# meyer-lab/cmtf-pls

Hardware: AMD Instinct MI355X
Metric: nipals_iters_per_sec (higher is better)
Workload: dtype f32

## Files before the change

### cmtf_pls_amd/_lib.py

```python
from __future__ import annotations

import ctypes
import os
from ctypes import c_char_p, c_double, c_int, c_int64, c_size_t, c_uint64, c_void_p

_HERE = os.path.dirname(os.path.abspath(__file__))
LIB_PATH = os.environ.get("CMTFPLS_LIB") or os.path.join(_HERE, "lib", "libcmtfpls.so")

_P = c_void_p

class XcovBlock(ctypes.Structure):
    _fields_ = [("S", _P), ("S2", _P), ("colcnt", _P), ("n_samples", c_double), ("order", c_int), ("A", c_int), ("B", c_int),
                ("n_squarings", c_int), ("Z", _P), ("wA", _P), ("wB", _P), ("info", _P)]


class KfoldState(ctypes.Structure):
    _fields_ = [("I", c_int), ("A", c_int), ("B", c_int), ("M", c_int), ("K", c_int), ("R", c_int)] + [
        (name, _P) for name in ("fold_of", "S", "mean", "Yk", "Gy", "WA", "WB", "Q", "Wa", "Wb", "T", "Gt", "coef", "Rm", "tm",
                                "Tout", "vec", "n_iter", "status", "part")]


SIGNATURES = {
    "cmtfpls_xcov_iterate_blocks_f64": (c_int, [ctypes.POINTER(XcovBlock), c_int, c_int, _P, _P, _P, _P, _P, c_int, _P, c_size_t, _P]),
    "cmtfpls_abi_version": (c_int, []),
    "cmtfpls_last_error": (c_char_p, []),
    "cmtfpls_clear_error": (c_int, []),
    "cmtfpls_status_to_host": (c_int, [_P, _P, c_size_t, _P, _P]),
    "cmtfpls_colstats_workspace_bytes": (c_size_t, [c_int64, c_int64]),
    "cmtfpls_colstats_f32": (c_int, [_P, c_int64, c_int64, _P, _P, _P, c_size_t, _P]),
    "cmtfpls_colstats_f64": (c_int, [_P, c_int64, c_int64, _P, _P, _P, c_size_t, _P]),
    "cmtfpls_sweep_partials": (c_int, []),
    "cmtfpls_center_f32": (c_int, [_P, c_int64, c_int64, _P, _P, _P, _P]),
    "cmtfpls_center_f64": (c_int, [_P, c_int64, c_int64, _P, _P, _P, _P]),
    "cmtfpls_mode0_contract_workspace_bytes": (c_size_t, [c_int64, c_int64]),
    "cmtfpls_mode0_contract_f32": (c_int, [_P, c_int64, c_int64, _P, _P, c_int, _P, c_size_t, _P]),
    "cmtfpls_mode0_contract_f64": (c_int, [_P, c_int64, c_int64, _P, _P, c_int, _P, c_size_t, _P]),
    "cmtfpls_mode0_contract_yq_f32": (c_int, [_P, c_int64, c_int64, _P, c_int, c_int, _P, _P, c_int, _P, c_size_t, _P]),
    "cmtfpls_mode0_contract_yq_f64": (c_int, [_P, c_int64, c_int64, _P, c_int, c_int, _P, _P, c_int, _P, c_size_t, _P]),
    "cmtfpls_colscale_f64": (c_int, [_P, c_int64, _P, c_double, _P]),
    "cmtfpls_rank1_workspace_bytes": (c_size_t, [c_int, c_int]),
    "cmtfpls_rank1_score_f64": (c_int, [_P, c_int, c_int, _P, _P, _P, c_int, _P, c_int, _P, _P, c_size_t, _P]),
    "cmtfpls_rank1_f64": (c_int, [_P, c_int, c_int, _P, _P, _P, _P, c_int, _P, c_size_t, _P]),
    "cmtfpls_rank1_launches_f64": (c_int, [_P, c_int, c_int, _P, _P, _P, _P, c_int, _P, c_size_t, _P]),
    "cmtfpls_rank1_chain_enable": (None, [c_int]),
    "cmtfpls_rank1_chain_enabled": (c_int, []),
    "cmtfpls_normalize_f64": (c_int, [_P, c_int64, _P, _P]),
    "cmtfpls_rank1_tensor_workspace_bytes": (c_size_t, [_P, c_int]),
    "cmtfpls_rank1_tensor_f64": (c_int, [_P, _P, c_int, c_double, _P, c_int, _P, c_int, _P, c_size_t, _P]),
    "cmtfpls_kron_f64": (c_int, [_P, c_int, _P, c_int, _P, _P]),
    "cmtfpls_xcov_workspace_bytes": (c_size_t, [c_int64, c_int64, c_int]),
    "cmtfpls_xcov_f32": (c_int, [_P, c_int64, c_int64, _P, c_int, c_int, _P, c_int, _P, c_size_t, _P]),
    "cmtfpls_xcov_f64": (c_int, [_P, c_int64, c_int64, _P, c_int, c_int, _P, c_int, _P, c_size_t, _P]),
    "cmtfpls_quadform_f64": (c_int, [_P, c_int, _P, _P, _P, _P]),
    "cmtfpls_xcov_iterate_f64": (c_int, [_P, c_int, c_int, c_int, _P, _P, _P, _P, _P, c_int, _P, _P, _P, c_int, _P, c_size_t, _P, c_size_t, _P]),
    "cmtfpls_s_downdate_f64": (c_int, [_P, c_int, c_int, c_int, _P, _P, _P, _P, _P, _P]),
    "cmtfpls_project_rows_f32": (c_int, [_P, c_int64, c_int, c_int, c_int, _P, _P, _P, _P, c_int, _P]),
    "cmtfpls_project_rows_f64": (c_int, [_P, c_int64, c_int, c_int, c_int, _P, _P, _P, _P, c_int, _P]),
    "cmtfpls_project_rows2_f32": (c_int, [_P, c_int, c_int, _P, _P, _P, _P, c_int, c_int, _P, _P, _P, c_int64, c_int, _P, c_int, _P]),
    "cmtfpls_project_rows2_f64": (c_int, [_P, c_int, c_int, _P, _P, _P, _P, c_int, c_int, _P, _P, _P, c_int64, c_int, _P, c_int, _P]),
    "cmtfpls_project_rows_idx_f32": (c_int, [_P, _P, c_int64, c_int, c_int, c_int, _P, _P, _P, _P, c_int, _P]),
    "cmtfpls_project_rows_idx_f64": (c_int, [_P, _P, c_int64, c_int, c_int, c_int, _P, _P, _P, _P, c_int, _P]),
    "cmtfpls_project_rows2_idx_f32": (c_int, [_P, c_int, c_int, _P, _P, _P, _P, c_int, c_int, _P, _P, _P, _P, c_int64, c_int, _P, c_int, _P]),
    "cmtfpls_project_rows2_idx_f64": (c_int, [_P, c_int, c_int, _P, _P, _P, _P, c_int, c_int, _P, _P, _P, _P, c_int64, c_int, _P, c_int, _P]),
    "cmtfpls_allreduce_sum_f64": (c_int, [_P, _P, c_size_t, _P]),
    "cmtfpls_allreduce_sum_f32": (c_int, [_P, _P, c_size_t, _P]),
    "cmtfpls_axpy_scalar_f64": (c_int, [_P, c_int64, _P, _P, _P]),
    "cmtfpls_xcov_deflate_f32": (c_int, [_P, c_int64, c_int, c_int, _P, c_int, c_int, _P, _P, _P, _P, _P, _P, c_size_t, _P]),
    "cmtfpls_xcov_deflate_f64": (c_int, [_P, c_int64, c_int, c_int, _P, c_int, c_int, _P, _P, _P, _P, _P, _P, c_size_t, _P]),
# ... 120 lines not shown
```

### cmtf_pls_amd/backend.py

```python
from __future__ import annotations

import ctypes
from typing import Optional, Tuple

import torch

from . import _lib

_SUFFIX = {torch.float32: "f32", torch.float64: "f64"}


def _ptr(t: Optional[torch.Tensor]):
    return None if t is None else t.data_ptr()


class HipBackend:
    name = "hip"

    def __init__(self, device: Optional[torch.device] = None):
        self.lib = _lib.load()
        if not torch.cuda.is_available():
            raise _lib.CmtfplsError("cmtf_pls_amd needs a ROCm GPU (torch.cuda.is_available() is False); there is no CPU fallback")
        self.device = torch.device(device) if device is not None else torch.device("cuda", torch.cuda.current_device())
        self.n_partials = int(self.lib.cmtfpls_sweep_partials())
        self._ws = {}
        self._status_slots = {}
        self.rank1_squarings = 30
        self.rank1_chain_side = 256 if self.lib.cmtfpls_rank1_chain_enabled() else 0

    def _stream(self):
        return torch.cuda.current_stream(self.device).cuda_stream

    def _workspace(self, key: str, nbytes: int) -> torch.Tensor:
        buf = self._ws.get(key)
        if buf is None or buf.numel() < nbytes:
            buf = torch.empty(max(int(nbytes), 256), dtype=torch.uint8, device=self.device)
            self._ws[key] = buf
        return buf

    def clear_error(self) -> bool:
        return bool(self.lib.cmtfpls_clear_error())

    def empty(self, *shape, dtype=torch.float64) -> torch.Tensor:
        return torch.empty(*shape, dtype=dtype, device=self.device)

    def zeros(self, *shape, dtype=torch.float64) -> torch.Tensor:
        return torch.zeros(*shape, dtype=dtype, device=self.device)

    def _fn(self, base: str, X: torch.Tensor):
        if X.dtype not in _SUFFIX:
            raise TypeError(f"X must be float32 or float64 on device, got {X.dtype}")
        assert X.is_contiguous() and X.device == self.device
        return getattr(self.lib, f"cmtfpls_{base}_{_SUFFIX[X.dtype]}")

    def _close_partials(self, part: torch.Tensor) -> torch.Tensor:
        out = self.empty(1)
        _lib.check(self.lib.cmtfpls_sum_f64(_ptr(part), part.numel(), _ptr(out), self._stream()), "sum")
        return out

    def ceiling(self, op: str, buf: torch.Tensor, row_bytes: int = 0, blocks: int = 2048,
# ... 31 lines not shown
    def mode0_contract(self, X2: torch.Tensor, u: torch.Tensor, masked: bool, out: Optional[torch.Tensor] = None) -> torch.Tensor:
        I, P = X2.shape
        ws = self._workspace("contract", self.lib.cmtfpls_mode0_contract_workspace_bytes(I, P))
        Z = out if out is not None else self.empty(P)
        _lib.check(self._fn("mode0_contract", X2)(_ptr(X2), I, P, _ptr(u), _ptr(Z), int(masked), _ptr(ws), ws.numel(), self._stream()), "mode0_contract")
        return Z

    def mode0_contract_yq(self, X2: torch.Tensor, Y: torch.Tensor, q: torch.Tensor, masked: bool,
                          out: torch.Tensor) -> Optional[torch.Tensor]:
        I, P = X2.shape
        ws = self._workspace("contract", self.lib.cmtfpls_mode0_contract_workspace_bytes(I, P))
        rc = self._fn("mode0_contract_yq", X2)(_ptr(X2), I, P, _ptr(Y), Y.stride(0), Y.shape[1], _ptr(q), _ptr(out), int(masked),
                                               _ptr(ws), ws.numel(), self._stream())
        if rc == 4:
            return None
        _lib.check(rc, "mode0_contract_yq")
        return out

    def colscale(self, Z: torch.Tensor, colcnt: torch.Tensor, n_samples: float) -> None:
        _lib.check(self.lib.cmtfpls_colscale_f64(_ptr(Z), Z.numel(), _ptr(colcnt), float(n_samples), self._stream()), "colscale")

    def rank1(self, Z: torch.Tensor, A: int, B: int, wA: torch.Tensor, wB: torch.Tensor,
              info: Optional[torch.Tensor] = None, n_squarings: Optional[int] = None, launches: bool = False) -> None:
        ws = self._workspace("rank1", self.lib.cmtfpls_rank1_workspace_bytes(A, B))
        fn = self.lib.cmtfpls_rank1_launches_f64 if launches else self.lib.cmtfpls_rank1_f64
        _lib.check(fn(_ptr(Z), A, B, _ptr(wA), _ptr(wB), None, _ptr(info), int(n_squarings or self.rank1_squarings),
                      _ptr(ws), ws.numel(), self._stream()), "rank1")

    def rank1_chain_gave_up(self) -> None:
        self.lib.cmtfpls_rank1_chain_enable(0)
        self.rank1_chain_side = 0

    def rank1_tensor(self, Z: torch.Tensor, dims, tol: float, factors: torch.Tensor,
                     info: Optional[torch.Tensor] = None, n_squarings: Optional[int] = None) -> None:
        import ctypes
        arr = (ctypes.c_int * len(dims))(*[int(d) for d in dims])
        ws = self._workspace("rank1t", self.lib.cmtfpls_rank1_tensor_workspace_bytes(arr, len(dims)))
        _lib.check(self.lib.cmtfpls_rank1_tensor_f64(_ptr(Z), arr, len(dims), float(tol), _ptr(factors), factors.stride(0), _ptr(info),
                                                     int(n_squarings or self.rank1_squarings), _ptr(ws), ws.numel(), self._stream()),
                   "rank1_tensor")

    def kron(self, a: torch.Tensor, b: torch.Tensor, out: torch.Tensor) -> torch.Tensor:
        _lib.check(self.lib.cmtfpls_kron_f64(_ptr(a), a.numel(), _ptr(b), b.numel(), _ptr(out), self._stream()), "kron")
        return out

    def normalize(self, v: torch.Tensor) -> None:
        _lib.check(self.lib.cmtfpls_normalize_f64(_ptr(v), v.numel(), None, self._stream()), "normalize")

    def xcov(self, X2: torch.Tensor, Y: torch.Tensor, masked: bool, out: Optional[torch.Tensor] = None,
             mixed: bool = False) -> Optional[torch.Tensor]:
        I, P = X2.shape
        M = Y.shape[1]
        ws = self._workspace("contract", self.lib.cmtfpls_xcov_workspace_bytes(I, P, M))
        S = out if out is not None else self.empty(M, P)
        fn = self.lib.cmtfpls_xcov_f32_mixed if (mixed and X2.dtype == torch.float32) else self._fn("xcov", X2)
        _lib.check(fn(_ptr(X2), I, P, _ptr(Y), Y.stride(0), M, _ptr(S), int(masked), _ptr(ws), ws.numel(), self._stream()), "xcov")
        return S

    def xcov_deflate(self, X2: torch.Tensor, A: int, B: int, Y: torch.Tensor, t: torch.Tensor, wA: torch.Tensor, wB: torch.Tensor,
                     out: torch.Tensor) -> Optional[torch.Tensor]:
        I, P = X2.shape
        M = Y.shape[1]
        if M > 64 or P % 4 != 0 or P != A * B:
            return None
        ws = self._workspace("contract", self.lib.cmtfpls_xcov_ssq_workspace_bytes(I, P, M))
        ssq = self.empty(1)
        rc = self._fn("xcov_deflate", X2)(_ptr(X2), I, A, B, _ptr(Y), Y.stride(0), M, _ptr(t), _ptr(wA), _ptr(wB), _ptr(out), _ptr(ssq),
                                          _ptr(ws), ws.numel(), self._stream())
        if rc == 4:
            return None
        _lib.check(rc, "xcov_deflate")
        return ssq

    def rank1_score(self, Z: torch.Tensor, A: int, B: int, wA: torch.Tensor, wB: torch.Tensor, S: torch.Tensor, tq: torch.Tensor,
                    info: Optional[torch.Tensor] = None, n_squarings: Optional[int] = None) -> torch.Tensor:
        M = S.shape[0]
        assert S.is_contiguous() and S.shape[1] == A * B and tq.numel() >= M
        ws = self._workspace("rank1", self.lib.cmtfpls_rank1_workspace_bytes(A, B))
        _lib.check(self.lib.cmtfpls_rank1_score_f64(_ptr(Z), A, B, _ptr(wA), _ptr(wB), _ptr(info),
                                                    int(n_squarings if n_squarings is not None else self.rank1_squarings),
                                                    _ptr(S), M, _ptr(tq), _ptr(ws), ws.numel(), self._stream()), "rank1_score")
        return tq

    def xcov_ssq(self, X2: torch.Tensor, Y: torch.Tensor, mean: torch.Tensor, out: torch.Tensor):
        I, P = X2.shape
        M = Y.shape[1]
        ws = self._workspace("contract", self.lib.cmtfpls_xcov_ssq_workspace_bytes(I, P, M))
        ssq = self.empty(1)
        assert mean.is_contiguous() and mean.numel() == P and mean.dtype == torch.float64
        _lib.check(self._fn("xcov_ssq", X2)(_ptr(X2), I, P, _ptr(Y), Y.stride(0), M, _ptr(out), _ptr(mean), _ptr(ssq), _ptr(ws), ws.numel(),
                                            self._stream()), "xcov_ssq")
        return out, ssq

    def xcov_stats(self, X2: torch.Tensor, Y: torch.Tensor, out: torch.Tensor):
        I, P = X2.shape
        M = Y.shape[1]
        if M > 64 or not X2.is_contiguous():
            return None
        ws = self._workspace("contract", self.lib.cmtfpls_xcov_stats_workspace_bytes(I, P, M))
        stats = self.empty(2 * P)
        rc = self._fn("xcov_stats", X2)(_ptr(X2), I, P, _ptr(Y), Y.stride(0), M, _ptr(out), _ptr(stats), _ptr(ws), ws.numel(), self._stream())
# ... 2 lines not shown
        _lib.check(rc, "xcov_stats")
        return out, stats

    def status_snapshot(self, status: torch.Tensor, slot: int, slots: Optional[dict] = None):
        slots = self._status_slots if slots is None else slots
        ent = slots.get((slot, status.numel()))
        if ent is None:
            host, ev = torch.empty(status.numel(), dtype=torch.float64, pin_memory=True), torch.cuda.Event()
            ev.record(torch.cuda.current_stream(self.device))
            ent = slots[(slot, status.numel())] = (host, ev, host.numpy(), host.data_ptr(), ev.cuda_event, status.numel() * 8)
        rc = self.lib.cmtfpls_status_to_host(status.data_ptr(), ent[3], ent[5], ent[4], self._stream())
        if rc:
            _lib.check(rc, "status_to_host")
        return ent

    def status_wait(self, token) -> "np.ndarray":
        token[1].synchronize()
        return token[2]

    def xcov_iterate_plan(self, S: torch.Tensor, A: int, B: int, q_cur: torch.Tensor, Z: torch.Tensor, wA: torch.Tensor,
                          wB: torch.Tensor, status: torch.Tensor, q_new: torch.Tensor, G: torch.Tensor):
        M, P = S.shape
        wc = self._workspace("contract", self.lib.cmtfpls_mode0_contract_workspace_bytes(M, P))
        wr = self._workspace("rank1", self.lib.cmtfpls_rank1_workspace_bytes(A, B))
        keep = (S, q_cur, Z, wA, wB, status, q_new, G, wc, wr)
        fn = self.lib.cmtfpls_xcov_iterate_f64
        head = (_ptr(S), M, A, B, _ptr(q_cur), _ptr(Z), _ptr(wA), _ptr(wB), status[1:3].data_ptr())
        tail = (_ptr(wc), wc.numel(), _ptr(wr), wr.numel())
        qn, Gp, du2 = _ptr(q_new), _ptr(G), status[0:1].data_ptr()
        stream = self._stream

        def enqueue(n_squarings: int, first: bool, _keep=keep) -> None:
            rc = fn(*head, n_squarings, qn, Gp, du2, 1 if first else 0, *tail, stream())
            if rc:
                _lib.check(rc, "xcov_iterate")
        return enqueue

    def xcov_iterate(self, S: torch.Tensor, A: int, B: int, q_cur: torch.Tensor, Z: torch.Tensor, wA: torch.Tensor,
                     wB: torch.Tensor, info: torch.Tensor, n_squarings: int, q_new: torch.Tensor, G: torch.Tensor,
                     du2: torch.Tensor, first: bool) -> None:
        M, P = S.shape
        wc = self._workspace("contract", self.lib.cmtfpls_mode0_contract_workspace_bytes(M, P))
        wr = self._workspace("rank1", self.lib.cmtfpls_rank1_workspace_bytes(A, B))
        _lib.check(self.lib.cmtfpls_xcov_iterate_f64(_ptr(S), M, A, B, _ptr(q_cur), _ptr(Z), _ptr(wA), _ptr(wB), _ptr(info),
                                                     int(n_squarings), _ptr(q_new), _ptr(G), _ptr(du2), int(first),
                                                     _ptr(wc), wc.numel(), _ptr(wr), wr.numel(), self._stream()), "xcov_iterate")

    def xcov_blocks_plan(self, blocks, M: int, q_cur: torch.Tensor, tq: torch.Tensor, q_new: torch.Tensor, G: torch.Tensor,
                         status: torch.Tensor):
        nb = len(blocks)
        if M > 64 or any(b["order"] not in (2, 3) for b in blocks) or tq.numel() != nb * M or not tq.is_contiguous():
            return None
        arr = (_lib.XcovBlock * nb)()
        need = 256
        for i, b in enumerate(blocks):
            for name in ("S", "S2", "colcnt", "Z", "wA", "wB"):
                t = b.get(name)
                assert t is None or (t.is_contiguous() and t.dtype == torch.float64 and t.device == self.device), name
                setattr(arr[i], name, _ptr(t))
            arr[i].n_samples, arr[i].order, arr[i].A, arr[i].B = float(b["n_samples"]), int(b["order"]), int(b["A"]), int(b["B"])
            arr[i].info = status[1 + 2 * i: 3 + 2 * i].data_ptr()
            if b["order"] == 3:
                need = max(need, self.lib.cmtfpls_rank1_workspace_bytes(b["A"], b["B"]))
        wr = self._workspace("rank1", need)
        keep = (blocks, q_cur, tq, q_new, G, status, wr, arr)
        fn, stream = self.lib.cmtfpls_xcov_iterate_blocks_f64, self._stream
# ... 519 lines not shown
```

### cmtf_pls_amd/csrc/rank1.hip

```cpp
#include "common.hpp"
#include <atomic>

namespace cmtfpls {

constexpr int kTile = 16;
constexpr int kMaxTiles = 256;
constexpr int kMaxSteps = 48;

struct Rank1Ctl {
  int done;
  int final_buf;
  int steps_used;
  int last_step;
  double pad[6];
};
__host__ __device__ __forceinline__ size_t rank1_ctl_bytes(int nt) {
  return sizeof(Rank1Ctl) + ((size_t)(kMaxSteps + 2) * nt + 2 * (size_t)nt * nt) * sizeof(double);
}
__device__ __forceinline__ double* ctl_trace(Rank1Ctl* c, int nt, int step) { return reinterpret_cast<double*>(c + 1) + (size_t)step * nt; }
__device__ __forceinline__ double* ctl_fro(Rank1Ctl* c, int nt, int which) {
  return reinterpret_cast<double*>(c + 1) + (size_t)(kMaxSteps + 2) * nt + (size_t)which * nt * nt;
}

__device__ __forceinline__ double pow2_scale_from_trace(const double* parts, int nt, double* tr_out) {
  double tr = 0.0;
  for (int i = 0; i < nt; ++i) tr += parts[i];
  *tr_out = tr;
  if (!(tr > 0.0) || !isfinite(tr)) return 1.0;
  int e;
  frexp(tr, &e);
  return ldexp(1.0, -e);
}

typedef double d4r_t __attribute__((ext_vector_type(4)));

__global__ __launch_bounds__(kTile* kTile) void syrk_step_kernel(const double* __restrict__ M, int n, int k, int ld,
                                                                double* __restrict__ C, Rank1Ctl* __restrict__ ctl,
// ... 112 lines not shown
      double t = 0.0;
      for (int l = 0; l < kTile; ++l) t += diag[l];
      ctl_trace(ctl, nt, step)[blockIdx.x] = t;
    }
  }
}

constexpr unsigned long long kChainEmpty = ~0ull;
constexpr int kChainMaxSteps = 31;
constexpr int kChainSpin = 1 << 15;

__device__ __forceinline__ double chain_ld(const double* p) {
  return __longlong_as_double((long long)__hip_atomic_load(reinterpret_cast<const unsigned long long*>(p), __ATOMIC_RELAXED, __HIP_MEMORY_SCOPE_AGENT));
}
__device__ __forceinline__ void chain_st(double* p, double v) {
  unsigned long long b = (unsigned long long)__double_as_longlong(v);
  if (b == kChainEmpty) b = 0x7FF8000000000000ull;
  __hip_atomic_store(reinterpret_cast<unsigned long long*>(p), b, __ATOMIC_RELAXED, __HIP_MEMORY_SCOPE_AGENT);
}
__device__ __forceinline__ bool chain_empty(double v) { return (unsigned long long)__double_as_longlong(v) == kChainEmpty; }

__global__ __launch_bounds__(256) void chain_preset_kernel(unsigned long long* __restrict__ p, int64_t n) {
  for (int64_t i = (int64_t)blockIdx.x * 256 + threadIdx.x; i < n; i += (int64_t)gridDim.x * 256) p[i] = kChainEmpty;
}

#ifdef CMTFPLS_CHAIN_PROFILE
__device__ unsigned long long g_chain_prof[1024];
#define CHAIN_STAMP(slot) do { if (first_wg && tid == 0 && step < 32) g_chain_prof[step * 8 + (slot)] = __builtin_amdgcn_s_memrealtime(); } while (0)
#define CHAIN_COUNT(slot, v) do { if (first_wg && tid == 0 && step < 32) g_chain_prof[step * 8 + (slot)] = (unsigned long long)(v); } while (0)
#else
#define CHAIN_STAMP(slot) do { } while (0)
#define CHAIN_COUNT(slot, v) do { } while (0)
#endif

__global__ __launch_bounds__(kTile* kTile) void syrk_chain_kernel(const double* __restrict__ M0, int n, int k0,
                                                                 double* gbufs, double* trs, double* fros, double* gave_up,
                                                                 Rank1Ctl* __restrict__ ctl, int n_squarings) {
  constexpr int KC = 128, KW = 8, LDP = KC + 2;
  __shared__ __attribute__((aligned(16))) double pan[2][kTile][LDP];
  __shared__ double red[2][4][kTile * kTile];
  __shared__ double diag[2][kTile];
  __shared__ double fsum[2][4];
  __shared__ double cfro[2][4];
  __shared__ double ctr[2][kTile];
  __shared__ int cdead[2];
  const int tx = threadIdx.x, ty = threadIdx.y, tid = ty * kTile + tx;
// ... 142 lines not shown
    __syncthreads();
    if (tid == 0) {
      chain_st(fros + (int64_t)step * nt2 + blockIdx.y * nt + blockIdx.x, ((fsum[par][0] + fsum[par][1]) + fsum[par][2]) + fsum[par][3]);
      if (blockIdx.x == blockIdx.y) {
        double t = 0.0;
        for (int l = 0; l < kTile; ++l) t += diag[par][l];
        chain_st(trs + (int64_t)step * nt + blockIdx.x, t);
      }
    }
    CHAIN_STAMP(6);
  }
}

__global__ __launch_bounds__(256) void transpose_kernel(const double* __restrict__ Z, int A, int B, double* __restrict__ Zt) {
  const int64_t idx = (int64_t)blockIdx.x * 256 + threadIdx.x;
  if (idx >= (int64_t)A * B) return;
  const int b = (int)(idx / A), a = (int)(idx % A);
  Zt[idx] = Z[(int64_t)a * B + b];
}

__global__ __launch_bounds__(256) void rank1_seed_xy_kernel(const double* __restrict__ M, int n, int k,
                                                           const double* __restrict__ gbase, int64_t gstride,
                                                           const double* __restrict__ G0,
                                                           const Rank1Ctl* __restrict__ ctl, int last_buf, int ny_blocks,
                                                           double* __restrict__ y, double* __restrict__ x) {
  extern __shared__ double seed[];
  __shared__ double red[16];
  __shared__ double rsum[8][33];
  __shared__ double bestv[4];
  __shared__ int besti[4];
  const int fb = (ctl->final_buf >= 0) ? ctl->final_buf : last_buf;
  const double* G = gbase + (int64_t)fb * gstride;
  double bv = -1.0;
  int bi = 0;
  for (int i = threadIdx.x; i < n; i += 256) {
    const double d = G[(int64_t)i * n + i];
    if (d > bv) { bv = d; bi = i; }
  }
#pragma unroll
  for (int m = 32; m > 0; m >>= 1) {
    const double ov = __shfl_xor(bv, m, 64);
    const int oi = __shfl_xor(bi, m, 64);
    if (ov > bv || (ov == bv && oi < bi)) { bv = ov; bi = oi; }
  }
  if ((threadIdx.x & 63) == 0) { bestv[threadIdx.x >> 6] = bv; besti[threadIdx.x >> 6] = bi; }
  __syncthreads();
  bv = bestv[0];
  bi = besti[0];
  for (int w = 1; w < 4; ++w)
    if (bestv[w] > bv || (bestv[w] == bv && besti[w] < bi)) { bv = bestv[w]; bi = besti[w]; }
  double ss = 0.0;
  for (int i = threadIdx.x; i < n; i += 256) {
    const double g = G[(int64_t)bi * n + i];
    seed[i] = g;
    ss = fma(g, g, ss);
// ... 9 lines not shown
      for (int i = lane; i < n; i += 64) s = fma(G0[(int64_t)j * n + i], seed[i], s);
      s = wave_sum(s);
      if (lane == 0) x[j] = s;
    }
    return;
  }
  const int cx = threadIdx.x & 31, ry = threadIdx.x >> 5;
  const int c = blockIdx.x * 32 + cx;
  double s = 0.0;
  if (c < k)
    for (int j = ry; j < n; j += 8) s = fma(M[(int64_t)j * k + c], seed[j], s);
  rsum[ry][cx] = s;
  __syncthreads();
  if (ry == 0 && c < k) {
    double tot = 0.0;
#pragma unroll
    for (int g = 0; g < 8; ++g) tot += rsum[g][cx];
    y[c] = tot;
  }
}

__device__ __forceinline__ void rank1_write_info(double* __restrict__ info, const Rank1Ctl* __restrict__ ctl, const double* gave) {
  if (!info) return;
  if (gave && !chain_empty(chain_ld(gave))) { info[0] = 0.0; info[1] = -1.0; return; }
  info[0] = (ctl->done || ctl->last_step >= 0) ? 1.0 : 0.0;
  info[1] = (double)ctl->steps_used;
}

__device__ __forceinline__ void rank1_final_body(const double* x, const double* y,
                                                 int n, int k, int x_is_A, const Rank1Ctl* __restrict__ ctl,
                                                 double* __restrict__ wA, double* __restrict__ wB,
                                                 double* __restrict__ sigma, double* __restrict__ info, const double* gave) {
  __shared__ double red[2][16];
  __shared__ double bestv[16];
  __shared__ int besti[16];
  double sx = 0.0, sy = 0.0;
  for (int i = threadIdx.x; i < n; i += 1024) sx = fma(x[i], x[i], sx);
  for (int i = threadIdx.x; i < k; i += 1024) sy = fma(y[i], y[i], sy);
  const double nx = sqrt(block_sum(sx, red[0]));
  const double ny = sqrt(block_sum(sy, red[1]));
  const double* vb = x_is_A ? y : x;
  const int nb = x_is_A ? k : n;
  double bv = -1.0;
  int bi = 0;
  for (int i = threadIdx.x; i < nb; i += 1024) {
    const double d = fabs(vb[i]);
    if (d > bv) { bv = d; bi = i; }
  }
#pragma unroll
  for (int m = 32; m > 0; m >>= 1) {
    const double ov = __shfl_xor(bv, m, 64);
    const int oi = __shfl_xor(bi, m, 64);
    if (ov > bv || (ov == bv && oi < bi)) { bv = ov; bi = oi; }
  }
  if ((threadIdx.x & 63) == 0) { bestv[threadIdx.x >> 6] = bv; besti[threadIdx.x >> 6] = bi; }
  __syncthreads();
  bv = bestv[0];
  bi = besti[0];
  for (int w = 1; w < 16; ++w)
    if (bestv[w] > bv || (bestv[w] == bv && besti[w] < bi)) { bv = bestv[w]; bi = besti[w]; }
  const bool gv = gave && !chain_empty(chain_ld(gave));
  const double sgn = gv ? __longlong_as_double(0x7FF8000000000000ll) : ((vb[bi] < 0.0) ? -1.0 : 1.0);
  double* ox = x_is_A ? wA : wB;
  double* oy = x_is_A ? wB : wA;
  for (int i = threadIdx.x; i < n; i += 1024) ox[i] = sgn * (x[i] / nx);
  for (int i = threadIdx.x; i < k; i += 1024) oy[i] = sgn * (y[i] / ny);
  if (threadIdx.x == 0) {
    if (sigma) sigma[0] = nx / ny;
    rank1_write_info(info, ctl, gave);
  }
}

__global__ __launch_bounds__(1024) void rank1_final_kernel(const double* __restrict__ x, const double* __restrict__ y,
                                                          int n, int k, int x_is_A, const Rank1Ctl* __restrict__ ctl,
                                                          double* __restrict__ wA, double* __restrict__ wB,
                                                          double* __restrict__ sigma, double* __restrict__ info, const double* gave) {
  rank1_final_body(x, y, n, k, x_is_A, ctl, wA, wB, sigma, info, gave);
}

__global__ __launch_bounds__(1024) void rank1_final_score_kernel(const double* __restrict__ x, const double* __restrict__ y,
                                                                int n, int k, int x_is_A, const Rank1Ctl* __restrict__ ctl,
                                                                double* __restrict__ wA, double* __restrict__ wB,
                                                                double* __restrict__ info, const double* __restrict__ S, int A, int B,
                                                                double* __restrict__ t, const double* gave) {
  extern __shared__ double lds[];
  __shared__ double red[2][16];
  __shared__ double bestv[16];
  __shared__ int besti[16];
  double* sA = lds;
  double* sB = lds + ((A + 1) & ~1);
  double sx = 0.0, sy = 0.0;
  for (int i = threadIdx.x; i < n; i += 1024) sx = fma(x[i], x[i], sx);
  for (int i = threadIdx.x; i < k; i += 1024) sy = fma(y[i], y[i], sy);
  const double nx = sqrt(block_sum(sx, red[0]));
  const double ny = sqrt(block_sum(sy, red[1]));
  const double* vb = x_is_A ? y : x;
  const int nb = x_is_A ? k : n;
  double bv = -1.0;
  int bi = 0;
  for (int i = threadIdx.x; i < nb; i += 1024) {
    const double d = fabs(vb[i]);
    if (d > bv) { bv = d; bi = i; }
  }
#pragma unroll
  for (int m = 32; m > 0; m >>= 1) {
    const double ov = __shfl_xor(bv, m, 64);
    const int oi = __shfl_xor(bi, m, 64);
    if (ov > bv || (ov == bv && oi < bi)) { bv = ov; bi = oi; }
  }
  if ((threadIdx.x & 63) == 0) { bestv[threadIdx.x >> 6] = bv; besti[threadIdx.x >> 6] = bi; }
  __syncthreads();
  bv = bestv[0];
  bi = besti[0];
  for (int w = 1; w < 16; ++w)
    if (bestv[w] > bv || (bestv[w] == bv && besti[w] < bi)) { bv = bestv[w]; bi = besti[w]; }
  const bool gv = gave && !chain_empty(chain_ld(gave));
  const double sgn = gv ? __longlong_as_double(0x7FF8000000000000ll) : ((vb[bi] < 0.0) ? -1.0 : 1.0);
  double* lx = x_is_A ? sA : sB;
  double* ly = x_is_A ? sB : sA;
  double* ox = x_is_A ? wA : wB;
  double* oy = x_is_A ? wB : wA;
  const bool store = blockIdx.x == 0;
  for (int i = threadIdx.x; i < n; i += 1024) {
    const double v = sgn * (x[i] / nx);
    lx[i] = v;
    if (store) ox[i] = v;
  }
  for (int i = threadIdx.x; i < k; i += 1024) {
    const double v = sgn * (y[i] / ny);
    ly[i] = v;
    if (store) oy[i] = v;
  }
  if (store && threadIdx.x == 0) rank1_write_info(info, ctl, gave);
  __syncthreads();
  using VT = Pack<double, 2>;
  const int64_t P = (int64_t)A * B;
  const int64_t step = (int64_t)1024 * 2;
  const double* __restrict__ xr = S + (int64_t)blockIdx.x * P;
  KronWalk w((int64_t)threadIdx.x * 2, step, B);
// ... 9 lines not shown
      double d = 0.0;
      d = fma(xs[u].e[0], sB[w.k], d);
      d = fma(xs[u].e[1], sB[w.k + 1], d);
      acc = fma(sA[w.j], d, acc);
      w.next();
    }
  }
  for (; c < P; c += step) {
    const VT xv = ld_stream(reinterpret_cast<const VT*>(xr + c));
    double d = 0.0;
    d = fma(xv.e[0], sB[w.k], d);
    d = fma(xv.e[1], sB[w.k + 1], d);
    acc = fma(sA[w.j], d, acc);
    w.next();
  }
  acc = block_sum(acc, red[0]);
  if (threadIdx.x == 0) t[blockIdx.x] = acc;
}

static inline size_t align_up(size_t x, size_t a) { return (x + a - 1) / a * a; }

static std::atomic<int> g_chain_on{1};

static int chain_slots() {
  static int slots = 0;
  if (slots == 0) {
    int dev = 0, cus = 0;
    if (hipGetDevice(&dev) != hipSuccess || hipDeviceGetAttribute(&cus, hipDeviceAttributeMultiprocessorCount, dev) != hipSuccess || cus <= 0) cus = 256;
    slots = 2 * cus;
  }
  return slots;
}

}

using namespace cmtfpls;

extern "C" {

size_t cmtfpls_rank1_workspace_bytes(int A, int B) {
  if (A <= 0 || B <= 0) return 0;
  const size_t n = (size_t)(A < B ? A : B), k = (size_t)(A < B ? B : A);
  const size_t nt = (n + kTile - 1) / kTile;
  const size_t chain = nt * nt <= 256 ? align_up(((size_t)(kChainMaxSteps + 1) * (n * n + nt + nt * nt) + 1) * sizeof(double), 256) : 0;
  return align_up(rank1_ctl_bytes((int)nt), 256) + 3 * align_up(n * n * sizeof(double), 256) +
         align_up((size_t)A * B * sizeof(double), 256) + align_up(n * sizeof(double), 256) + align_up(k * sizeof(double), 256) + chain;
}

static int rank1_run(const double* Z, int A, int B, double* wA, double* wB, double* sigma, double* info,
                     int n_squarings, void* ws, size_t ws_bytes, void* stream, const double* S, int M, double* tq, bool allow_chain = true);

int cmtfpls_rank1_f64(const double* Z, int A, int B, double* wA, double* wB, double* sigma, double* info,
                      int n_squarings, void* ws, size_t ws_bytes, void* stream) {
  return rank1_run(Z, A, B, wA, wB, sigma, info, n_squarings, ws, ws_bytes, stream, nullptr, 0, nullptr);
}

#ifdef CMTFPLS_CHAIN_PROFILE
int cmtfpls_debug_chain_prof(unsigned long long* out) { return (int)hipMemcpyFromSymbol(out, HIP_SYMBOL(g_chain_prof), sizeof(unsigned long long) * 1024); }
#endif
void cmtfpls_rank1_chain_enable(int on) { g_chain_on.store((on == 1 || on == 2) ? on : 0, std::memory_order_relaxed); }
int cmtfpls_rank1_chain_enabled(void) { return g_chain_on.load(std::memory_order_relaxed); }

int cmtfpls_rank1_launches_f64(const double* Z, int A, int B, double* wA, double* wB, double* sigma, double* info,
                               int n_squarings, void* ws, size_t ws_bytes, void* stream) {
  return rank1_run(Z, A, B, wA, wB, sigma, info, n_squarings, ws, ws_bytes, stream, nullptr, 0, nullptr, false);
}

int cmtfpls_rank1_score_f64(const double* Z, int A, int B, double* wA, double* wB, double* info, int n_squarings,
                            const double* S, int M, double* tq, void* ws, size_t ws_bytes, void* stream) {
  if (!S || !tq || M <= 0) { set_error("rank1_score: bad argument"); return CMTFPLS_EINVAL; }
  const int64_t P = (int64_t)A * B;
  if (M > 64 || P < 8192 || (B % 2) != 0 || ((size_t)(((A + 1) & ~1) + B) * sizeof(double)) > 60 * 1024 ||
      (reinterpret_cast<uintptr_t>(S) & 15) != 0) {
    int rc = cmtfpls_rank1_f64(Z, A, B, wA, wB, nullptr, info, n_squarings, ws, ws_bytes, stream);
    if (rc == CMTFPLS_OK) rc = cmtfpls_score_s_f64(S, M, A, B, wA, wB, tq, stream);
    return rc;
  }
  return rank1_run(Z, A, B, wA, wB, nullptr, info, n_squarings, ws, ws_bytes, stream, S, M, tq);
}

static int rank1_run(const double* Z, int A, int B, double* wA, double* wB, double* sigma, double* info,
                     int n_squarings, void* ws, size_t ws_bytes, void* stream, const double* S, int M, double* tq, bool allow_chain) {
  if (!Z || !wA || !wB || A <= 0 || B <= 0) { set_error("rank1: bad argument"); return CMTFPLS_EINVAL; }
  const int n = A < B ? A : B, k = A < B ? B : A;
  if (n > kTile * kMaxTiles) { set_error("rank1: min(A, B) > 4096 unsupported"); return CMTFPLS_EUNSUPPORTED; }
  if ((size_t)n * sizeof(double) > 64 * 1024) { set_error("rank1: seed exceeds the LDS"); return CMTFPLS_EUNSUPPORTED; }
  if (n_squarings < 1) n_squarings = 1;
  if (n_squarings > kMaxSteps) n_squarings = kMaxSteps;
  if (!ws || ws_bytes < cmtfpls_rank1_workspace_bytes(A, B)) { set_error("rank1: workspace too small"); return CMTFPLS_EWORKSPACE; }
  hipStream_t st = (hipStream_t)stream;
  char* p = static_cast<char*>(ws);
  Rank1Ctl* ctl = reinterpret_cast<Rank1Ctl*>(p);
  p += align_up(rank1_ctl_bytes((n + kTile - 1) / kTile), 256);
  double* buf0 = reinterpret_cast<double*>(p);
  p += align_up((size_t)n * n * sizeof(double), 256);
  double* buf1 = reinterpret_cast<double*>(p);
  p += align_up((size_t)n * n * sizeof(double), 256);
  double* g0keep = reinterpret_cast<double*>(p);
  p += align_up((size_t)n * n * sizeof(double), 256);
  double* Zt = reinterpret_cast<double*>(p);
  p += align_up((size_t)A * B * sizeof(double), 256);
  double* xv = reinterpret_cast<double*>(p);
  p += align_up((size_t)n * sizeof(double), 256);
  double* yv = reinterpret_cast<double*>(p);
  p += align_up((size_t)k * sizeof(double), 256);
  double* chain_region = reinterpret_cast<double*>(p);

  const double* M0 = Z;
  if (A > B) {
    const int64_t tot = (int64_t)A * B;
    hipLaunchKernelGGL(transpose_kernel, dim3((unsigned)((tot + 255) / 256)), dim3(256), 0, st, Z, A, B, Zt);
    M0 = Zt;
  }
  const int nt = (n + kTile - 1) / kTile;
  const dim3 grid(nt, nt), block(kTile, kTile);
  const int ny_blocks = (k + 31) / 32;
  const double* gave = nullptr;
  if (allow_chain && g_chain_on.load(std::memory_order_relaxed) && nt * nt <= 256 && nt * nt <= chain_slots() && n_squarings <= kChainMaxSteps) {
    const size_t nn = (size_t)n * n, steps = (size_t)n_squarings + 1;
    double* gbufs = chain_region;
    double* trs = gbufs + steps * nn;
    double* fros = trs + steps * nt;
    double* gave_up = fros + steps * (size_t)nt * nt;
    gave = gave_up;
    const int64_t words = (int64_t)(steps * (nn + nt + (size_t)nt * nt) + 1);
    hipLaunchKernelGGL(chain_preset_kernel, dim3((unsigned)((words + 2047) / 2048)), dim3(256), 0, st, reinterpret_cast<unsigned long long*>(chain_region), words);
    const dim3 cgrid(nt, (g_chain_on.load(std::memory_order_relaxed) == 2 && nt > 1) ? nt - 1 : nt);
    hipLaunchKernelGGL(syrk_chain_kernel, cgrid, block, 0, st, M0, n, k, gbufs, trs, fros, gave_up, ctl, n_squarings);
    hipLaunchKernelGGL(rank1_seed_xy_kernel, dim3(ny_blocks + (n + 3) / 4), dim3(256), (size_t)n * sizeof(double), st,
                       M0, n, k, gbufs, (int64_t)nn, gbufs, ctl, n_squarings, ny_blocks, yv, xv);
  } else {
    hipLaunchKernelGGL(syrk_step_kernel, grid, block, 0, st, M0, n, k, k, buf0, ctl, 0, 0, g0keep);
    for (int s = 1; s <= n_squarings; ++s) {
      const double* in = (s & 1) ? buf0 : buf1;
      double* out = (s & 1) ? buf1 : buf0;
      hipLaunchKernelGGL(syrk_step_kernel, grid, block, 0, st, in, n, n, n, out, ctl, s, s & 1, (double*)nullptr);
    }
    hipLaunchKernelGGL(rank1_seed_xy_kernel, dim3(ny_blocks + (n + 3) / 4), dim3(256), (size_t)n * sizeof(double), st,
                       M0, n, k, buf0, (int64_t)(buf1 - buf0), g0keep, ctl, n_squarings & 1, ny_blocks, yv, xv);
  }
  if (S) {
    const size_t lds = (size_t)(((A + 1) & ~1) + B) * sizeof(double);
    hipLaunchKernelGGL(rank1_final_score_kernel, dim3((unsigned)M), dim3(1024), lds, st, xv, yv, n, k, (A <= B) ? 1 : 0, ctl, wA, wB, info,
                       S, A, B, tq, gave);
    return check_launch("rank1_score");
  }
  hipLaunchKernelGGL(rank1_final_kernel, dim3(1), dim3(1024), 0, st, xv, yv, n, k, (A <= B) ? 1 : 0, ctl, wA, wB, sigma, info, gave);
  return check_launch("rank1");
}

}
```

### include/cmtfpls.h

```cpp
#ifndef CMTFPLS_H
#define CMTFPLS_H

#include <stddef.h>
#include <stdint.h>

#ifdef __cplusplus
extern "C" {
#endif

#define CMTFPLS_OK 0
#define CMTFPLS_EINVAL 1
#define CMTFPLS_EWORKSPACE 2
#define CMTFPLS_EHIP 3
#define CMTFPLS_EUNSUPPORTED 4

int cmtfpls_abi_version(void);
const char* cmtfpls_last_error(void);
int cmtfpls_clear_error(void);
int cmtfpls_status_to_host(const void* src, void* dst_host, size_t bytes, void* event, void* stream);

size_t cmtfpls_colstats_workspace_bytes(int64_t I, int64_t P);
int cmtfpls_colstats_f32(const float* X, int64_t I, int64_t P, double* colsum, double* colcnt,
                         void* ws, size_t ws_bytes, void* stream);
int cmtfpls_colstats_f64(const double* X, int64_t I, int64_t P, double* colsum, double* colcnt,
// ... 2 lines not shown
int cmtfpls_center_f32(float* X, int64_t I, int64_t P, const double* mean, double* rowcnt,
                       double* ssq_part, void* stream);
int cmtfpls_center_f64(double* X, int64_t I, int64_t P, const double* mean, double* rowcnt,
                       double* ssq_part, void* stream);

size_t cmtfpls_mode0_contract_workspace_bytes(int64_t I, int64_t P);
int cmtfpls_mode0_contract_f32(const float* X, int64_t I, int64_t P, const double* u, double* Z,
                               int masked, void* ws, size_t ws_bytes, void* stream);
int cmtfpls_mode0_contract_f64(const double* X, int64_t I, int64_t P, const double* u, double* Z,
                               int masked, void* ws, size_t ws_bytes, void* stream);
int cmtfpls_mode0_contract_yq_f32(const float* X, int64_t I, int64_t P, const double* Y, int ldy, int M,
                                  const double* q, double* Z, int masked, void* ws, size_t ws_bytes, void* stream);
int cmtfpls_mode0_contract_yq_f64(const double* X, int64_t I, int64_t P, const double* Y, int ldy, int M,
                                  const double* q, double* Z, int masked, void* ws, size_t ws_bytes, void* stream);
int cmtfpls_colscale_f64(double* Z, int64_t P, const double* colcnt, double n_samples, void* stream);

size_t cmtfpls_rank1_workspace_bytes(int A, int B);
int cmtfpls_rank1_f64(const double* Z, int A, int B, double* wA, double* wB, double* sigma, double* info,
                      int n_squarings, void* ws, size_t ws_bytes, void* stream);
int cmtfpls_rank1_launches_f64(const double* Z, int A, int B, double* wA, double* wB, double* sigma, double* info,
                               int n_squarings, void* ws, size_t ws_bytes, void* stream);
void cmtfpls_rank1_chain_enable(int on);
int cmtfpls_rank1_chain_enabled(void);
int cmtfpls_rank1_score_f64(const double* Z, int A, int B, double* wA, double* wB, double* info, int n_squarings,
                            const double* S, int M, double* tq, void* ws, size_t ws_bytes, void* stream);
int cmtfpls_normalize_f64(double* v, int64_t n, double* nrm, void* stream);
size_t cmtfpls_rank1_tensor_workspace_bytes(const int* dims, int n);
int cmtfpls_rank1_tensor_f64(const double* Z, const int* dims, int n, double tol, double* factors, int ld,
                             double* info, int n_squarings, void* ws, size_t ws_bytes, void* stream);
int cmtfpls_kron_f64(const double* a, int na, const double* b, int nb, double* out, void* stream);

size_t cmtfpls_xcov_workspace_bytes(int64_t I, int64_t P, int M);
int cmtfpls_xcov_f32(const float* X, int64_t I, int64_t P, const double* Y, int ldy, int M, double* S,
                     int masked, void* ws, size_t ws_bytes, void* stream);
int cmtfpls_xcov_f64(const double* X, int64_t I, int64_t P, const double* Y, int ldy, int M, double* S,
                     int masked, void* ws, size_t ws_bytes, void* stream);
int cmtfpls_quadform_f64(const double* G, int M, const double* q, const double* q_old, double* out, void* stream);
int cmtfpls_xcov_deflate_f32(float* X, int64_t I, int A, int B, const double* Y, int ldy, int M, const double* t, const double* wA,
                             const double* wB, double* S, double* ssq, void* ws, size_t ws_bytes, void* stream);
int cmtfpls_xcov_deflate_f64(double* X, int64_t I, int A, int B, const double* Y, int ldy, int M, const double* t, const double* wA,
                             const double* wB, double* S, double* ssq, void* ws, size_t ws_bytes, void* stream);
size_t cmtfpls_xcov_ssq_workspace_bytes(int64_t I, int64_t P, int M);
size_t cmtfpls_xcov_stats_workspace_bytes(int64_t I, int64_t P, int M);
int cmtfpls_xcov_stats_f32(const float* X, int64_t I, int64_t P, const double* Y, int ldy, int M, double* S, double* stats,
                           void* ws, size_t ws_bytes, void* stream);
int cmtfpls_xcov_stats_f64(const double* X, int64_t I, int64_t P, const double* Y, int ldy, int M, double* S, double* stats,
// ... 233 lines not shown
```

Measured before the change: 765.6.

## Carry chain-region reset into rank1 final kernel to skip preset launch

Rank1 workspaces are now registered per shape, and the chain-region reset (writing the empty sentinel) is done by extra blocks appended to the final/score kernel. The next call on the same workspace can then skip the separate chain_preset_kernel launch. The gave-up flag is latched into the control block by the seed kernel, because the final kernel now overwrites the region that flag lives in. This removes one kernel launch per rank1 call on the hot NIPALS path, at the cost of host-side mutex/map bookkeeping, special handling under graph capture, and a one-shape-per-workspace restriction.

```diff
diff --git a/cmtf_pls_amd/_lib.py b/cmtf_pls_amd/_lib.py
--- a/cmtf_pls_amd/_lib.py
+++ b/cmtf_pls_amd/_lib.py
@@ -44,6 +44,10 @@
     "cmtfpls_rank1_launches_f64": (c_int, [_P, c_int, c_int, _P, _P, _P, _P, c_int, _P, c_size_t, _P]),
     "cmtfpls_rank1_chain_enable": (None, [c_int]),
     "cmtfpls_rank1_chain_enabled": (c_int, []),
+    "cmtfpls_rank1_workspace_register": (c_int, [_P]),
+    "cmtfpls_rank1_workspace_release": (c_int, [_P]),
+    "cmtfpls_rank1_preset_carry_enable": (None, [c_int]),
+    "cmtfpls_rank1_preset_carry_enabled": (c_int, []),
     "cmtfpls_normalize_f64": (c_int, [_P, c_int64, _P, _P]),
     "cmtfpls_rank1_tensor_workspace_bytes": (c_size_t, [_P, c_int]),
     "cmtfpls_rank1_tensor_f64": (c_int, [_P, _P, c_int, c_double, _P, c_int, _P, c_int, _P, c_size_t, _P]),
diff --git a/cmtf_pls_amd/backend.py b/cmtf_pls_amd/backend.py
--- a/cmtf_pls_amd/backend.py
+++ b/cmtf_pls_amd/backend.py
@@ -1,6 +1,7 @@
 from __future__ import annotations
 
 import ctypes
+import weakref
 from typing import Optional, Tuple
 
 import torch
@@ -12,6 +13,11 @@
 
 def _ptr(t: Optional[torch.Tensor]):
     return None if t is None else t.data_ptr()
+
+
+def _release_rank1_workspaces(lib, ptrs) -> None:
+    for ptr in ptrs:
+        lib.cmtfpls_rank1_workspace_release(ptr)
 
 
 class HipBackend:
@@ -27,6 +33,8 @@
         self._status_slots = {}
         self.rank1_squarings = 30
         self.rank1_chain_side = 256 if self.lib.cmtfpls_rank1_chain_enabled() else 0
+        self._rank1_registered = []
+        weakref.finalize(self, _release_rank1_workspaces, self.lib, self._rank1_registered)
 
     def _stream(self):
         return torch.cuda.current_stream(self.device).cuda_stream
@@ -36,6 +44,15 @@
         if buf is None or buf.numel() < nbytes:
             buf = torch.empty(max(int(nbytes), 256), dtype=torch.uint8, device=self.device)
             self._ws[key] = buf
+        return buf
+
+    def _rank1_workspace(self, A: int, B: int) -> torch.Tensor:
+        key = ("rank1", int(A), int(B))
+        buf = self._ws.get(key)
+        if buf is None:
+            buf = self._ws[key] = torch.empty(max(int(self.lib.cmtfpls_rank1_workspace_bytes(A, B)), 256), dtype=torch.uint8, device=self.device)
+            _lib.check(self.lib.cmtfpls_rank1_workspace_register(buf.data_ptr()), "rank1_workspace_register")
+            self._rank1_registered.append(buf.data_ptr())
         return buf
 
     def clear_error(self) -> bool:
@@ -113,7 +130,7 @@
 
     def rank1(self, Z: torch.Tensor, A: int, B: int, wA: torch.Tensor, wB: torch.Tensor,
               info: Optional[torch.Tensor] = None, n_squarings: Optional[int] = None, launches: bool = False) -> None:
-        ws = self._workspace("rank1", self.lib.cmtfpls_rank1_workspace_bytes(A, B))
+        ws = self._rank1_workspace(A, B)
         fn = self.lib.cmtfpls_rank1_launches_f64 if launches else self.lib.cmtfpls_rank1_f64
         _lib.check(fn(_ptr(Z), A, B, _ptr(wA), _ptr(wB), None, _ptr(info), int(n_squarings or self.rank1_squarings),
                       _ptr(ws), ws.numel(), self._stream()), "rank1")
@@ -121,6 +138,8 @@
     def rank1_chain_gave_up(self) -> None:
         self.lib.cmtfpls_rank1_chain_enable(0)
         self.rank1_chain_side = 0
+        for ptr in self._rank1_registered:
+            self.lib.cmtfpls_rank1_workspace_register(ptr)
 
     def rank1_tensor(self, Z: torch.Tensor, dims, tol: float, factors: torch.Tensor,
                      info: Optional[torch.Tensor] = None, n_squarings: Optional[int] = None) -> None:
@@ -167,7 +186,7 @@
                     info: Optional[torch.Tensor] = None, n_squarings: Optional[int] = None) -> torch.Tensor:
         M = S.shape[0]
         assert S.is_contiguous() and S.shape[1] == A * B and tq.numel() >= M
-        ws = self._workspace("rank1", self.lib.cmtfpls_rank1_workspace_bytes(A, B))
+        ws = self._rank1_workspace(A, B)
         _lib.check(self.lib.cmtfpls_rank1_score_f64(_ptr(Z), A, B, _ptr(wA), _ptr(wB), _ptr(info),
                                                     int(n_squarings if n_squarings is not None else self.rank1_squarings),
                                                     _ptr(S), M, _ptr(tq), _ptr(ws), ws.numel(), self._stream()), "rank1_score")
@@ -216,7 +235,7 @@
                           wB: torch.Tensor, status: torch.Tensor, q_new: torch.Tensor, G: torch.Tensor):
         M, P = S.shape
         wc = self._workspace("contract", self.lib.cmtfpls_mode0_contract_workspace_bytes(M, P))
-        wr = self._workspace("rank1", self.lib.cmtfpls_rank1_workspace_bytes(A, B))
+        wr = self._rank1_workspace(A, B)
         keep = (S, q_cur, Z, wA, wB, status, q_new, G, wc, wr)
         fn = self.lib.cmtfpls_xcov_iterate_f64
         head = (_ptr(S), M, A, B, _ptr(q_cur), _ptr(Z), _ptr(wA), _ptr(wB), status[1:3].data_ptr())
@@ -235,7 +254,7 @@
                      du2: torch.Tensor, first: bool) -> None:
         M, P = S.shape
         wc = self._workspace("contract", self.lib.cmtfpls_mode0_contract_workspace_bytes(M, P))
-        wr = self._workspace("rank1", self.lib.cmtfpls_rank1_workspace_bytes(A, B))
+        wr = self._rank1_workspace(A, B)
         _lib.check(self.lib.cmtfpls_xcov_iterate_f64(_ptr(S), M, A, B, _ptr(q_cur), _ptr(Z), _ptr(wA), _ptr(wB), _ptr(info),
                                                      int(n_squarings), _ptr(q_new), _ptr(G), _ptr(du2), int(first),
                                                      _ptr(wc), wc.numel(), _ptr(wr), wr.numel(), self._stream()), "xcov_iterate")
diff --git a/cmtf_pls_amd/csrc/rank1.hip b/cmtf_pls_amd/csrc/rank1.hip
--- a/cmtf_pls_amd/csrc/rank1.hip
+++ b/cmtf_pls_amd/csrc/rank1.hip
@@ -1,5 +1,7 @@
 #include "common.hpp"
 #include <atomic>
+#include <mutex>
+#include <unordered_map>
 
 namespace cmtfpls {
 
@@ -12,7 +14,9 @@
   int final_buf;
   int steps_used;
   int last_step;
-  double pad[6];
+  int gave_seen;
+  int pad_i;
+  double pad[5];
 };
 __host__ __device__ __forceinline__ size_t rank1_ctl_bytes(int nt) {
   return sizeof(Rank1Ctl) + ((size_t)(kMaxSteps + 2) * nt + 2 * (size_t)nt * nt) * sizeof(double);
@@ -171,6 +175,15 @@
 
 __global__ __launch_bounds__(256) void chain_preset_kernel(unsigned long long* __restrict__ p, int64_t n) {
   for (int64_t i = (int64_t)blockIdx.x * 256 + threadIdx.x; i < n; i += (int64_t)gridDim.x * 256) p[i] = kChainEmpty;
+}
+
+__device__ __forceinline__ void chain_represet(unsigned long long* __restrict__ p, int64_t n, int first) {
+  const int64_t stride = (int64_t)(gridDim.x - first) * blockDim.x;
+  for (int64_t i = (int64_t)((int)blockIdx.x - first) * blockDim.x + threadIdx.x; i < n; i += stride) p[i] = kChainEmpty;
+}
+__host__ __device__ __forceinline__ int chain_represet_blocks(int64_t words) {
+  const int64_t b = (words + 4095) / 4096;
+  return (int)(b < 1 ? 1 : (b > 128 ? 128 : b));
 }
 
 #ifdef CMTFPLS_CHAIN_PROFILE
@@ -359,8 +372,8 @@
 __global__ __launch_bounds__(256) void rank1_seed_xy_kernel(const double* __restrict__ M, int n, int k,
                                                            const double* __restrict__ gbase, int64_t gstride,
                                                            const double* __restrict__ G0,
-                                                           const Rank1Ctl* __restrict__ ctl, int last_buf, int ny_blocks,
-                                                           double* __restrict__ y, double* __restrict__ x) {
+                                                           Rank1Ctl* __restrict__ ctl, int last_buf, int ny_blocks,
+                                                           double* __restrict__ y, double* __restrict__ x, const double* gave) {
   extern __shared__ double seed[];
   __shared__ double red[16];
   __shared__ double rsum[8][33];
@@ -368,6 +381,7 @@
   __shared__ int besti[4];
   const int fb = (ctl->final_buf >= 0) ? ctl->final_buf : last_buf;
   const double* G = gbase + (int64_t)fb * gstride;
+  if (blockIdx.x == 0 && threadIdx.x == 0) ctl->gave_seen = (gave && !chain_empty(chain_ld(gave))) ? 1 : 0;
   double bv = -1.0;
   int bi = 0;
   for (int i = threadIdx.x; i < n; i += 256) {
@@ -423,7 +437,7 @@
 
 __device__ __forceinline__ void rank1_write_info(double* __restrict__ info, const Rank1Ctl* __restrict__ ctl, const double* gave) {
   if (!info) return;
-  if (gave && !chain_empty(chain_ld(gave))) { info[0] = 0.0; info[1] = -1.0; return; }
+  if (gave && ctl->gave_seen) { info[0] = 0.0; info[1] = -1.0; return; }
   info[0] = (ctl->done || ctl->last_step >= 0) ? 1.0 : 0.0;
   info[1] = (double)ctl->steps_used;
 }
@@ -460,7 +474,7 @@
   bi = besti[0];
   for (int w = 1; w < 16; ++w)
     if (bestv[w] > bv || (bestv[w] == bv && besti[w] < bi)) { bv = bestv[w]; bi = besti[w]; }
-  const bool gv = gave && !chain_empty(chain_ld(gave));
+  const bool gv = gave && ctl->gave_seen;
   const double sgn = gv ? __longlong_as_double(0x7FF8000000000000ll) : ((vb[bi] < 0.0) ? -1.0 : 1.0);
   double* ox = x_is_A ? wA : wB;
   double* oy = x_is_A ? wB : wA;
@@ -475,7 +489,9 @@
 __global__ __launch_bounds__(1024) void rank1_final_kernel(const double* __restrict__ x, const double* __restrict__ y,
                                                           int n, int k, int x_is_A, const Rank1Ctl* __restrict__ ctl,
                                                           double* __restrict__ wA, double* __restrict__ wB,
-                                                          double* __restrict__ sigma, double* __restrict__ info, const double* gave) {
+                                                          double* __restrict__ sigma, double* __restrict__ info, const double* gave,
+                                                          unsigned long long* __restrict__ region, int64_t region_words) {
+  if (blockIdx.x > 0) { chain_represet(region, region_words, 1); return; }
   rank1_final_body(x, y, n, k, x_is_A, ctl, wA, wB, sigma, info, gave);
 }
 
@@ -483,7 +499,9 @@
                                                                 int n, int k, int x_is_A, const Rank1Ctl* __restrict__ ctl,
                                                                 double* __restrict__ wA, double* __restrict__ wB,
                                                                 double* __restrict__ info, const double* __restrict__ S, int A, int B,
-                                                                double* __restrict__ t, const double* gave) {
+                                                                double* __restrict__ t, const double* gave, int M,
+                                                                unsigned long long* __restrict__ region, int64_t region_words) {
+  if ((int)blockIdx.x >= M) { chain_represet(region, region_words, M); return; }
   extern __shared__ double lds[];
   __shared__ double red[2][16];
   __shared__ double bestv[16];
@@ -515,7 +533,7 @@
   bi = besti[0];
   for (int w = 1; w < 16; ++w)
     if (bestv[w] > bv || (bestv[w] == bv && besti[w] < bi)) { bv = bestv[w]; bi = besti[w]; }
-  const bool gv = gave && !chain_empty(chain_ld(gave));
+  const bool gv = gave && ctl->gave_seen;
   const double sgn = gv ? __longlong_as_double(0x7FF8000000000000ll) : ((vb[bi] < 0.0) ? -1.0 : 1.0);
   double* lx = x_is_A ? sA : sB;
   double* ly = x_is_A ? sB : sA;
@@ -571,6 +589,11 @@
 
 static std::atomic<int> g_chain_on{1};
 
+static std::atomic<int> g_preset_carry{1};
+struct CarryState { int A, B; int64_t words; };
+static std::mutex g_carry_mu;
+static std::unordered_map<const void*, CarryState> g_carry;
+
 static int chain_slots() {
   static int slots = 0;
   if (slots == 0) {
@@ -609,6 +632,19 @@
 #endif
 void cmtfpls_rank1_chain_enable(int on) { g_chain_on.store((on == 1 || on == 2) ? on : 0, std::memory_order_relaxed); }
 int cmtfpls_rank1_chain_enabled(void) { return g_chain_on.load(std::memory_order_relaxed); }
+void cmtfpls_rank1_preset_carry_enable(int on) { g_preset_carry.store(on ? 1 : 0, std::memory_order_relaxed); }
+int cmtfpls_rank1_preset_carry_enabled(void) { return g_preset_carry.load(std::memory_order_relaxed); }
+int cmtfpls_rank1_workspace_register(const void* ws) {
+  if (!ws) { set_error("rank1_workspace_register: bad argument"); return CMTFPLS_EINVAL; }
+  std::lock_guard<std::mutex> lk(g_carry_mu);
+  g_carry[ws] = CarryState{0, 0, 0};
+  return CMTFPLS_OK;
+}
+int cmtfpls_rank1_workspace_release(const void* ws) {
+  std::lock_guard<std::mutex> lk(g_carry_mu);
+  g_carry.erase(ws);
+  return CMTFPLS_OK;
+}
 
 int cmtfpls_rank1_launches_f64(const double* Z, int A, int B, double* wA, double* wB, double* sigma, double* info,
                                int n_squarings, void* ws, size_t ws_bytes, void* stream) {
@@ -628,6 +664,15 @@
   return rank1_run(Z, A, B, wA, wB, nullptr, info, n_squarings, ws, ws_bytes, stream, S, M, tq);
 }
 
+static int carry_checked(int rc, const void* ws) {
+  if (rc != CMTFPLS_OK) {
+    std::lock_guard<std::mutex> lk(g_carry_mu);
+    auto it = g_carry.find(ws);
+    if (it != g_carry.end()) it->second.words = 0;
+  }
+  return rc;
+}
+
 static int rank1_run(const double* Z, int A, int B, double* wA, double* wB, double* sigma, double* info,
                      int n_squarings, void* ws, size_t ws_bytes, void* stream, const double* S, int M, double* tq, bool allow_chain) {
   if (!Z || !wA || !wB || A <= 0 || B <= 0) { set_error("rank1: bad argument"); return CMTFPLS_EINVAL; }
@@ -637,6 +682,14 @@
   if (n_squarings < 1) n_squarings = 1;
   if (n_squarings > kMaxSteps) n_squarings = kMaxSteps;
   if (!ws || ws_bytes < cmtfpls_rank1_workspace_bytes(A, B)) { set_error("rank1: workspace too small"); return CMTFPLS_EWORKSPACE; }
+  {
+    std::lock_guard<std::mutex> lk(g_carry_mu);
+    auto it = g_carry.find(ws);
+    if (it != g_carry.end()) {
+      if (it->second.A == 0) { it->second.A = A; it->second.B = B; }
+      else if (it->second.A != A || it->second.B != B) { set_error("rank1: a registered workspace serves one shape"); return CMTFPLS_EINVAL; }
+    }
+  }
   hipStream_t st = (hipStream_t)stream;
   char* p = static_cast<char*>(ws);
   Rank1Ctl* ctl = reinterpret_cast<Rank1Ctl*>(p);
@@ -665,6 +718,7 @@
   const dim3 grid(nt, nt), block(kTile, kTile);
   const int ny_blocks = (k + 31) / 32;
   const double* gave = nullptr;
+  int64_t carry_words = 0;
   if (allow_chain && g_chain_on.load(std::memory_order_relaxed) && nt * nt <= 256 && nt * nt <= chain_slots() && n_squarings <= kChainMaxSteps) {
     const size_t nn = (size_t)n * n, steps = (size_t)n_squarings + 1;
     double* gbufs = chain_region;
@@ -673,11 +727,24 @@
     double* gave_up = fros + steps * (size_t)nt * nt;
     gave = gave_up;
     const int64_t words = (int64_t)(steps * (nn + nt + (size_t)nt * nt) + 1);
-    hipLaunchKernelGGL(chain_preset_kernel, dim3((unsigned)((words + 2047) / 2048)), dim3(256), 0, st, reinterpret_cast<unsigned long long*>(chain_region), words);
+    bool preset = true;
+    {
+      std::lock_guard<std::mutex> lk(g_carry_mu);
+      auto it = g_carry.find(ws);
+      if (it != g_carry.end()) {
+        carry_words = words;
+        preset = !(g_preset_carry.load(std::memory_order_relaxed) && it->second.words >= words);
+        hipStreamCaptureStatus cap = hipStreamCaptureStatusNone;
+        if (hipStreamIsCapturing(st, &cap) != hipSuccess) { (void)hipGetLastError(); cap = hipStreamCaptureStatusActive; }
+        if (cap == hipStreamCaptureStatusNone && it->second.words < words) it->second.words = words;
+      }
+    }
+    if (preset)
+      hipLaunchKernelGGL(chain_preset_kernel, dim3((unsigned)((words + 2047) / 2048)), dim3(256), 0, st, reinterpret_cast<unsigned long long*>(chain_region), words);
     const dim3 cgrid(nt, (g_chain_on.load(std::memory_order_relaxed) == 2 && nt > 1) ? nt - 1 : nt);
     hipLaunchKernelGGL(syrk_chain_kernel, cgrid, block, 0, st, M0, n, k, gbufs, trs, fros, gave_up, ctl, n_squarings);
     hipLaunchKernelGGL(rank1_seed_xy_kernel, dim3(ny_blocks + (n + 3) / 4), dim3(256), (size_t)n * sizeof(double), st,
-                       M0, n, k, gbufs, (int64_t)nn, gbufs, ctl, n_squarings, ny_blocks, yv, xv);
+                       M0, n, k, gbufs, (int64_t)nn, gbufs, ctl, n_squarings, ny_blocks, yv, xv, gave);
   } else {
     hipLaunchKernelGGL(syrk_step_kernel, grid, block, 0, st, M0, n, k, k, buf0, ctl, 0, 0, g0keep);
     for (int s = 1; s <= n_squarings; ++s) {
@@ -686,16 +753,19 @@
       hipLaunchKernelGGL(syrk_step_kernel, grid, block, 0, st, in, n, n, n, out, ctl, s, s & 1, (double*)nullptr);
     }
     hipLaunchKernelGGL(rank1_seed_xy_kernel, dim3(ny_blocks + (n + 3) / 4), dim3(256), (size_t)n * sizeof(double), st,
-                       M0, n, k, buf0, (int64_t)(buf1 - buf0), g0keep, ctl, n_squarings & 1, ny_blocks, yv, xv);
-  }
+                       M0, n, k, buf0, (int64_t)(buf1 - buf0), g0keep, ctl, n_squarings & 1, ny_blocks, yv, xv, gave);
+  }
+  unsigned long long* region = carry_words > 0 ? reinterpret_cast<unsigned long long*>(chain_region) : nullptr;
+  const int extra = carry_words > 0 ? chain_represet_blocks(carry_words) : 0;
   if (S) {
     const size_t lds = (size_t)(((A + 1) & ~1) + B) * sizeof(double);
-    hipLaunchKernelGGL(rank1_final_score_kernel, dim3((unsigned)M), dim3(1024), lds, st, xv, yv, n, k, (A <= B) ? 1 : 0, ctl, wA, wB, info,
-                       S, A, B, tq, gave);
-    return check_launch("rank1_score");
-  }
-  hipLaunchKernelGGL(rank1_final_kernel, dim3(1), dim3(1024), 0, st, xv, yv, n, k, (A <= B) ? 1 : 0, ctl, wA, wB, sigma, info, gave);
-  return check_launch("rank1");
-}
-
-}
+    hipLaunchKernelGGL(rank1_final_score_kernel, dim3((unsigned)(M + extra)), dim3(1024), lds, st, xv, yv, n, k, (A <= B) ? 1 : 0, ctl, wA, wB, info,
+                       S, A, B, tq, gave, M, region, carry_words);
+    return carry_checked(check_launch("rank1_score"), ws);
+  }
+  hipLaunchKernelGGL(rank1_final_kernel, dim3((unsigned)(1 + extra)), dim3(1024), 0, st, xv, yv, n, k, (A <= B) ? 1 : 0, ctl, wA, wB, sigma, info, gave,
+                     region, carry_words);
+  return carry_checked(check_launch("rank1"), ws);
+}
+
+}
diff --git a/include/cmtfpls.h b/include/cmtfpls.h
--- a/include/cmtfpls.h
+++ b/include/cmtfpls.h
@@ -48,6 +48,10 @@
                                int n_squarings, void* ws, size_t ws_bytes, void* stream);
 void cmtfpls_rank1_chain_enable(int on);
 int cmtfpls_rank1_chain_enabled(void);
+int cmtfpls_rank1_workspace_register(const void* ws);
+int cmtfpls_rank1_workspace_release(const void* ws);
+void cmtfpls_rank1_preset_carry_enable(int on);
+int cmtfpls_rank1_preset_carry_enabled(void);
 int cmtfpls_rank1_score_f64(const double* Z, int A, int B, double* wA, double* wB, double* info, int n_squarings,
                             const double* S, int M, double* tq, void* ws, size_t ws_bytes, void* stream);
 int cmtfpls_normalize_f64(double* v, int64_t n, double* nrm, void* stream);
```

After: 767.2, median of 6. About the same (+0.2%).
